# Illumina/canvas

Measured on AMD Instinct MI355X. Metric: genome-bins/sec (bin+clean+partition), higher is better.
Workload: dtype u8/int32 (bin), f32/f64 (clean, viterbi); 1 GPU; BASELINE configs[2]: whole-genome GRCh38 60x single sample, full bin+clean+partition HIP path on 1 MI355X per sample; bins_after_clean=4686240, bin_size=534, partition=PerSampleHMM, clean_flags=-g -s -r --local-sd-metric-file, segments=250, samples=1

## Files before the change

### canvas_amd/csrc/hmm.hip

```cpp
#include "common.hpp"
#include <type_traits>
#include "select.hpp"
#include "quantize.hpp"
#include <mutex>
#include <cmath>
#include <thread>
#include <cstring>
#include <limits>
#include <algorithm>

#define NSTATE 5

struct HmmParams {
    double logA[NSTATE][NSTATE];
    double logPi[NSTATE];
    int32_t tableLen;
    double maxThreshold;
};

__global__ void __launch_bounds__(256) k_keys_cov_f32(const double* __restrict__ cov, int64_t n, uint32_t* __restrict__ keys) {
    int64_t i = (int64_t)blockIdx.x * 256 + threadIdx.x;
    if (i < n) keys[i] = key_of_float((float)cov[i]);
}

// ... 232 lines not shown
            e = eNext;
        }
        __syncthreads();
        if (l < steps)
            psi[C.begin + t0 + l] = (uint16_t)(sPsi[0][l] | (sPsi[1][l] << 3) | (sPsi[2][l] << 6) | (sPsi[3][l] << 9) | (sPsi[4][l] << 12));
        __syncthreads();
    }
    double d[NSTATE];
#pragma unroll
    for (int i = 0; i < NSTATE; i++) d[i] = readlane_f64(delta, i);
    if (l == 0) {
        int best = -1; double m1 = NEG;
#pragma unroll
        for (int i = 0; i < NSTATE; i++) if (d[i] > m1) { best = i; m1 = d[i]; }
        lastState[cidx] = best;
    }
}


#define VB 128
#define VW0 16
#define VW 128
#define VW2 64
#define PQ 8
#define MAP_IDENT (0u | (1u << 3) | (2u << 6) | (3u << 9) | (4u << 12))
struct VitBlock { int32_t chrom; int32_t t0; };
struct __attribute__((aligned(4))) VecI4 { int v[4]; };
struct __attribute__((aligned(8))) VecD2 { double v[2]; };
struct __attribute__((aligned(2))) VecH8 { uint32_t w[4]; };

template <int J, bool TWO = false>
__device__ __forceinline__ void vit_state(const double (&d)[NSTATE], double e, const HmmParams& P, double& outDelta, uint32_t& outArg) {
    const double NEG = -1.7976931348623157e308;
    const double cOff = e + P.logA[J == 0 ? 1 : 0][J], cDiag = e + P.logA[J][J];
    const double t_0 = d[0] + (TWO ? (J == 0 ? cDiag : cOff) : (e + P.logA[0][J]));
    const double t_1 = d[1] + (TWO ? (J == 1 ? cDiag : cOff) : (e + P.logA[1][J]));
    const double t_2 = d[2] + (TWO ? (J == 2 ? cDiag : cOff) : (e + P.logA[2][J]));
    const double t_3 = d[3] + (TWO ? (J == 3 ? cDiag : cOff) : (e + P.logA[3][J]));
    const double t_4 = d[4] + (TWO ? (J == 4 ? cDiag : cOff) : (e + P.logA[4][J]));
    double a = __builtin_fmax(__builtin_fmax(__builtin_fmax(t_0, t_1), __builtin_fmax(t_2, t_3)), t_4);
    uint32_t ia = t_3 == a ? 3u : 4u;
    ia = t_2 == a ? 2u : ia; ia = t_1 == a ? 1u : ia; ia = t_0 == a ? 0u : ia;
    if (!(a > NEG)) { a = NEG; ia = 0; }
    outDelta = a; outArg = ia;
}
template <bool TWO = false>
__device__ __forceinline__ uint32_t vit_step5(double (&d)[NSTATE], const double (&e)[NSTATE], const HmmParams& P) {
    double n0, n1, n2, n3, n4; uint32_t a0, a1, a2, a3, a4;
    vit_state<0, TWO>(d, e[0], P, n0, a0); vit_state<1, TWO>(d, e[1], P, n1, a1); vit_state<2, TWO>(d, e[2], P, n2, a2);
    vit_state<3, TWO>(d, e[3], P, n3, a3); vit_state<4, TWO>(d, e[4], P, n4, a4);
    d[0] = n0; d[1] = n1; d[2] = n2; d[3] = n3; d[4] = n4;
    return a0 | (a1 << 3) | (a2 << 6) | (a3 << 9) | (a4 << 12);
}
__device__ __forceinline__ void vit_init5(double (&d)[NSTATE], const double (&e)[NSTATE], const HmmParams& P) {
#pragma unroll
    for (int j = 0; j < NSTATE; j++) { double lik = e[j] + P.logA[0][j]; d[j] = P.logPi[j] + lik - P.logA[0][j]; }
}
__device__ __forceinline__ int vit_best5(const double (&d)[NSTATE]) {
    int best = -1; double m1 = -1.7976931348623157e308;
#pragma unroll
    for (int i = 0; i < NSTATE; i++) if (d[i] > m1) { best = i; m1 = d[i]; }
    return best;
}
__device__ __forceinline__ uint32_t map_get(uint32_t m, uint32_t j) { return (m >> (3u * j)) & 7u; }
__device__ __forceinline__ uint32_t map_compose(uint32_t outer, uint32_t inner) {
    return map_get(outer, map_get(inner, 0)) | (map_get(outer, map_get(inner, 1)) << 3) | (map_get(outer, map_get(inner, 2)) << 6) |
           (map_get(outer, map_get(inner, 3)) << 9) | (map_get(outer, map_get(inner, 4)) << 12);
}
__device__ __forceinline__ double sel5(const double (&d)[NSTATE], uint32_t i) {
    double r = d[0];
    r = i == 1 ? d[1] : r; r = i == 2 ? d[2] : r; r = i == 3 ? d[3] : r; r = i == 4 ? d[4] : r;
    return r;
}
__device__ __forceinline__ void vit_emissions(double (&e)[NSTATE], const double* __restrict__ sTab, const double* __restrict__ logPmf, bool useLds, int tableLen, int k) {
    if (useLds) {
#pragma unroll
        for (int j = 0; j < NSTATE; j++) e[j] = sTab[k * NSTATE + j];
    } else {
#pragma unroll
        for (int j = 0; j < NSTATE; j++) e[j] = logPmf[(size_t)j * tableLen + k];
    }
}
__device__ __forceinline__ void vit_stage_table(double* sTab, const double* __restrict__ logPmf, int tableLen, bool useLds) {
    if (useLds) for (int i = threadIdx.x; i < tableLen * NSTATE; i += blockDim.x) { int s = i / tableLen, k = i - s * tableLen; sTab[k * NSTATE + s] = logPmf[i]; }
    __syncthreads();
}
__device__ __forceinline__ int wave_max_i32(int v) {
#pragma unroll
    for (int d = 32; d >= 1; d >>= 1) { int o = __shfl_xor(v, d); v = o > v ? o : v; }
    return v;
}

template <typename T>
__global__ void __launch_bounds__(256) k_make_blocks(const int32_t* __restrict__ first, int nchr, int n, int per, T* __restrict__ out) {
    const int i = blockIdx.x * 256 + threadIdx.x;
    if (i >= n) return;
    int lo = 0, hi = nchr - 1;
    while (lo < hi) { int mid = (lo + hi + 1) >> 1; if (first[mid] <= i) lo = mid; else hi = mid - 1; }
    while (lo < nchr - 1 && first[lo + 1] <= i) lo++;
    T b; b.chrom = lo; b.t0 = (i - first[lo]) * per;
    out[i] = b;
}

template <typename T> __device__ __forceinline__ void make_block_entry(const int32_t* __restrict__ first, int nchr, int i, int per, T* __restrict__ out) {
    int lo = 0, hi = nchr - 1;
    while (lo < hi) { int mid = (lo + hi + 1) >> 1; if (first[mid] <= i) lo = mid; else hi = mid - 1; }
    while (lo < nchr - 1 && first[lo + 1] <= i) lo++;
    T b; b.chrom = lo; b.t0 = (i - first[lo]) * per;
    out[i] = b;
}
#define HMM_BYVAL 64
struct HmmDescPack { HmmChrom chroms[HMM_BYVAL]; int64_t off[HMM_BYVAL + 1]; int32_t first[HMM_BYVAL + 1], firstChunk[HMM_BYVAL + 1], firstS[HMM_BYVAL + 1], firstGroup[HMM_BYVAL + 1]; };
struct HmmDescDev { HmmChrom* chroms; int64_t* off; int32_t* first; int32_t* firstChunk; int32_t* firstS; int32_t* firstGroup; };
template <typename VB_T, typename BB_T>
__global__ void __launch_bounds__(256) k_hmm_setup(const HmmDescPack pack, int usePack, HmmDescDev D, int nchr,
                                                   int nblocks, int nblocksS, int nchunks, int vb, int vbs, int bbChunk, VB_T* __restrict__ vBlocks, VB_T* __restrict__ sBlocks, BB_T* __restrict__ bChunks,
                                                   const double* __restrict__ cov, int64_t N, double maxThreshold, int32_t* __restrict__ idx, int32_t* __restrict__ dLast, int32_t* __restrict__ dFail) {
    const int32_t* first = usePack ? pack.first : D.first; const int32_t* firstS = usePack ? pack.firstS : D.firstS; const int32_t* firstChunk = usePack ? pack.firstChunk : D.firstChunk;
    if (usePack && blockIdx.x == 0) {
        for (int c = threadIdx.x; c < nchr; c += 256) D.chroms[c] = pack.chroms[c];
        for (int c = threadIdx.x; c <= nchr; c += 256) { D.off[c] = pack.off[c]; D.first[c] = pack.first[c]; D.firstChunk[c] = pack.firstChunk[c]; D.firstS[c] = pack.firstS[c]; D.firstGroup[c] = pack.firstGroup[c]; }
    }
    const int64_t i = (int64_t)blockIdx.x * 256 + threadIdx.x;
    if (i < nblocks) make_block_entry(first, nchr, (int)i, vb, vBlocks);
    if (i < nblocksS) make_block_entry(firstS, nchr, (int)i, vbs, sBlocks);
    if (i < nchunks) make_block_entry(firstChunk, nchr, (int)i, bbChunk, bChunks);
    if (i < nchr) { dLast[i] = -1; dFail[i] = 0; }
    if (cov && i < N) {
        double x = cov[i];
        x = x > maxThreshold ? maxThreshold : x;
        const int32_t k = (int32_t)rint(x);
        idx[i] = k < 0 ? 0 : k;
    }
}

template <bool useLds, bool TWO>
__global__ void __launch_bounds__(64) k_vit_spec(const VitBlock* __restrict__ blocks, int nblocks, const HmmChrom* __restrict__ chroms, const int32_t* __restrict__ idx,
                                                 const double* __restrict__ logPmf, HmmParams P, uint16_t* __restrict__ psi, uint16_t* __restrict__ maps,
                                                 int32_t* __restrict__ lastGuess, int leadIn, const int32_t* __restrict__ todo, int vb) {
    extern __shared__ double sTab[];
    vit_stage_table(sTab, logPmf, P.tableLen, useLds);
    const int b = blockIdx.x * 64 + threadIdx.x;
    const bool actBlock = b < nblocks;
    const VitBlock B = blocks[actBlock ? b : nblocks - 1];
    const HmmChrom C = chroms[B.chrom];
    const int64_t tBeg = B.t0, tEnd = (B.t0 + vb < C.T) ? B.t0 + vb : C.T;
    const int64_t ts = tBeg > leadIn ? tBeg - leadIn : 0;
    const bool act = actBlock && (!todo || todo[B.chrom]);
    const int nsteps = act ? (int)(tEnd - ts) : 0;
    const int maxSteps = wave_max_i32(nsteps);
    const int32_t* __restrict__ ix = idx + C.begin + ts;
    uint16_t* __restrict__ pp = psi + C.begin;
    double d[NSTATE] = {0.0, 0.0, 0.0, 0.0, 0.0};
    uint32_t fm = MAP_IDENT;
    const int lead = (int)(tBeg - ts);
    if (nsteps > 0) {
        double e[NSTATE];
        vit_emissions(e, sTab, logPmf, useLds, P.tableLen, ix[0]);
        if (ts == 0) vit_init5(d, e, P);
        else {
#pragma unroll
            for (int j = 0; j < NSTATE; j++) d[j] = e[j];
        }
        if (lead == 0) pp[ts] = 0;
    }
    VecI4 qa = *reinterpret_cast<const VecI4*>(ix + 1), qb = *reinterpret_cast<const VecI4*>(ix + 5);
    double eCur[NSTATE];
// ... 446 lines not shown
    double r = x0;
    r = p == 1 ? x1 : r; r = p == 2 ? x2 : r; r = p == 3 ? x3 : r; r = p == 4 ? x4 : r;
    return r;
}
struct VerState { double d[NSTATE]; uint32_t valid; bool bad; double Dprev; int sPrev; uint32_t why; };
template <bool useLds>
__device__ __forceinline__ void ver_lead_step(VerState& S, const LogA25& A, const double* __restrict__ sTab, const double* __restrict__ logPmf, int tableLen,
                                              bool on, int k, int sCur, double v, uint32_t pk) {
    double e[NSTATE];
    vit_emissions(e, sTab, logPmf, useLds, tableLen, on ? k : 0);
    const double Dt = S.Dprev + v;
    double nd[NSTATE]; uint32_t nv = 0;
    const double la5[NSTATE] = {pick5(map_get(pk, 0), LOGA_COL(A, 0)), pick5(map_get(pk, 1), LOGA_COL(A, 1)), pick5(map_get(pk, 2), LOGA_COL(A, 2)),
                                pick5(map_get(pk, 3), LOGA_COL(A, 3)), pick5(map_get(pk, 4), LOGA_COL(A, 4))};
#pragma unroll
    for (int j = 0; j < NSTATE; j++) {
        const uint32_t p = map_get(pk, j);
        const double dp = pick5(p, S.d[0], S.d[1], S.d[2], S.d[3], S.d[4]);
        const bool vp = ((S.valid >> p) & 1u) != 0;
        const double step = e[j] + la5[j];
        const bool isCur = j == sCur, fromPrev = (int)p == S.sPrev;
        const double viaPrev = S.Dprev + step, viaAnc = dp + step;
        const double r0 = vp ? viaAnc : S.d[j], r1 = fromPrev ? viaPrev : r0, r = isCur ? Dt : r1;
        nd[j] = r; nv |= (isCur || fromPrev || vp) ? (1u << j) : 0u;
    }
#pragma unroll
    for (int j = 0; j < NSTATE; j++) S.d[j] = on ? nd[j] : S.d[j];
    S.valid = on ? nv : S.valid; S.Dprev = on ? Dt : S.Dprev; S.sPrev = on ? sCur : S.sPrev;
}
template <bool useLds>
__device__ __forceinline__ void ver_block_step(VerState& S, const HmmParams& P, const double* __restrict__ sTab, const double* __restrict__ logPmf, bool on, int k, int sCur,
                                               double v, uint32_t pk) {
    double e[NSTATE], dn[NSTATE];
    vit_emissions(e, sTab, logPmf, useLds, P.tableLen, on ? k : 0);
    const double Dt = S.Dprev + v;
#pragma unroll
    for (int j = 0; j < NSTATE; j++) dn[j] = S.d[j];
    const uint32_t got = vit_step5(dn, e, P);
    S.bad = S.bad || (on && (S.valid != 31u || got != pk || sel5(dn, (uint32_t)(on ? sCur : 0)) != Dt));
    S.why |= on ? ((S.valid != 31u ? 2u : 0u) | (got != pk ? 4u : 0u) | (sel5(dn, (uint32_t)(on ? sCur : 0)) != Dt ? 8u : 0u)) : 0u;
#pragma unroll
    for (int j = 0; j < NSTATE; j++) S.d[j] = on ? dn[j] : S.d[j];
    S.Dprev = on ? Dt : S.Dprev; S.sPrev = on ? sCur : S.sPrev;
}
template <bool useLds, bool LEAD>
__device__ __forceinline__ void ver_phase(VerState& S, const LogA25& A, const HmmParams& P, const double* __restrict__ sTab, const double* __restrict__ logPmf,
                                          const int32_t* __restrict__ ixp, const int32_t* __restrict__ stp, const double* __restrict__ vp, const uint16_t* __restrict__ ppp, int cnt) {
    const int maxCnt = wave_max_i32(cnt);
    int kq[PQ], sq[PQ]; double vq[PQ]; uint32_t pq[PQ];
#pragma unroll
    for (int u = 0; u < PQ; u++) { const bool in = u < cnt; kq[u] = in ? ixp[u] : 0; sq[u] = in ? stp[u] : 0; vq[u] = in ? vp[u] : 0.0; pq[u] = in ? ppp[u] : 0u; }
    for (int j0 = 0; j0 < maxCnt; j0 += PQ) {
        int kn[PQ], sn[PQ]; double vn[PQ]; VecH8 pn;
        if (j0 + 2 * PQ <= cnt) {
            const int o = j0 + PQ;
            const VecI4 ka = *reinterpret_cast<const VecI4*>(ixp + o), kb = *reinterpret_cast<const VecI4*>(ixp + o + 4);
            const VecI4 sa = *reinterpret_cast<const VecI4*>(stp + o), sb = *reinterpret_cast<const VecI4*>(stp + o + 4);
            const VecD2 v0 = *reinterpret_cast<const VecD2*>(vp + o), v1 = *reinterpret_cast<const VecD2*>(vp + o + 2), v2 = *reinterpret_cast<const VecD2*>(vp + o + 4),
                        v3 = *reinterpret_cast<const VecD2*>(vp + o + 6);
            pn = *reinterpret_cast<const VecH8*>(ppp + o);
#pragma unroll
            for (int u = 0; u < 4; u++) { kn[u] = ka.v[u]; kn[4 + u] = kb.v[u]; sn[u] = sa.v[u]; sn[4 + u] = sb.v[u]; }
            vn[0] = v0.v[0]; vn[1] = v0.v[1]; vn[2] = v1.v[0]; vn[3] = v1.v[1]; vn[4] = v2.v[0]; vn[5] = v2.v[1]; vn[6] = v3.v[0]; vn[7] = v3.v[1];
        } else {
#pragma unroll
            for (int u = 0; u < PQ; u++) { const bool in = j0 + PQ + u < cnt; kn[u] = in ? ixp[j0 + PQ + u] : 0; sn[u] = in ? stp[j0 + PQ + u] : 0; vn[u] = in ? vp[j0 + PQ + u] : 0.0; }
#pragma unroll
            for (int u = 0; u < 4; u++) pn.w[u] = (uint32_t)(j0 + PQ + 2 * u < cnt ? ppp[j0 + PQ + 2 * u] : (uint16_t)0) | ((uint32_t)(j0 + PQ + 2 * u + 1 < cnt ? ppp[j0 + PQ + 2 * u + 1] : (uint16_t)0) << 16);
        }
#pragma unroll
        for (int u = 0; u < PQ; u++) {
            if (LEAD) ver_lead_step<useLds>(S, A, sTab, logPmf, P.tableLen, j0 + u < cnt, kq[u], sq[u], vq[u], pq[u]);
            else ver_block_step<useLds>(S, P, sTab, logPmf, j0 + u < cnt, kq[u], sq[u], vq[u], pq[u]);
        }
        __builtin_amdgcn_sched_barrier(0);
#pragma unroll
        for (int u = 0; u < PQ; u++) { kq[u] = kn[u]; sq[u] = sn[u]; vq[u] = vn[u]; pq[u] = (pn.w[u >> 1] >> (16 * (u & 1))) & 0xFFFFu; }
    }
}
template <bool useLds>
__global__ void __launch_bounds__(64) k_vit_verify(const VitBlock* __restrict__ blocks, int nblocks, const HmmChrom* __restrict__ chroms, const int32_t* __restrict__ idx,
                                                   const double* __restrict__ logPmf, HmmParams P, const uint16_t* __restrict__ psi,
                                                   const int32_t* __restrict__ state, const double* __restrict__ V, const double* __restrict__ carry, const int32_t* __restrict__ lastGuess,
                                                   int32_t* __restrict__ fail, int leadIn, const int32_t* __restrict__ todo) {
    extern __shared__ double sTab[];
    vit_stage_table(sTab, logPmf, P.tableLen, useLds);
    const int b = blockIdx.x * 64 + threadIdx.x;
    const bool actBlock = b < nblocks;
    const VitBlock B = blocks[actBlock ? b : nblocks - 1];
    const HmmChrom C = chroms[B.chrom];
    const int64_t tBeg = B.t0, tEnd = (B.t0 + VB < C.T) ? B.t0 + VB : C.T;
    const int64_t ts = tBeg > leadIn ? tBeg - leadIn : 0;
    const bool act = actBlock && (!todo || todo[B.chrom]);
    const int nsteps = act ? (int)(tEnd - ts) : 0;
    const int maxSteps = wave_max_i32(nsteps);
    const int32_t* __restrict__ ix = idx + C.begin + ts;
    const int32_t* __restrict__ st = state + C.begin + ts;
    const double* __restrict__ Vc = V + C.begin + ts;
    const uint16_t* __restrict__ pp = psi + C.begin + ts;
    VerState S;
#pragma unroll
    for (int j = 0; j < NSTATE; j++) S.d[j] = 0.0;
    S.valid = 0; S.bad = false; S.why = 0;
    S.Dprev = carry[C.begin + ts];
    S.sPrev = ts > 0 ? state[C.begin + ts - 1] : -1;
    LogA25 A;
#define LOGA_LOAD(i, j) A.a##i##j = P.logA[i][j]; asm volatile("" : "+v"(A.a##i##j));
    LOGA_LOAD(0, 0) LOGA_LOAD(0, 1) LOGA_LOAD(0, 2) LOGA_LOAD(0, 3) LOGA_LOAD(0, 4) LOGA_LOAD(1, 0) LOGA_LOAD(1, 1) LOGA_LOAD(1, 2) LOGA_LOAD(1, 3) LOGA_LOAD(1, 4)
    LOGA_LOAD(2, 0) LOGA_LOAD(2, 1) LOGA_LOAD(2, 2) LOGA_LOAD(2, 3) LOGA_LOAD(2, 4) LOGA_LOAD(3, 0) LOGA_LOAD(3, 1) LOGA_LOAD(3, 2) LOGA_LOAD(3, 3) LOGA_LOAD(3, 4)
    LOGA_LOAD(4, 0) LOGA_LOAD(4, 1) LOGA_LOAD(4, 2) LOGA_LOAD(4, 3) LOGA_LOAD(4, 4)
#undef LOGA_LOAD
    const int lead = (int)(tBeg - ts);
    if (nsteps > 0) {
        if (ts == 0) {
            double e[NSTATE];
            vit_emissions(e, sTab, logPmf, useLds, P.tableLen, ix[0]);
            const double Dt = S.Dprev + Vc[0];
            const int sCur = st[0];
            vit_init5(S.d, e, P); S.valid = 31u;
            if (sel5(S.d, (uint32_t)sCur) != Dt) { S.bad = true; S.why |= 16u; }
            S.Dprev = Dt; S.sPrev = sCur;
        } else ver_lead_step<useLds>(S, A, sTab, logPmf, P.tableLen, true, ix[0], st[0], Vc[0], (uint32_t)pp[0]);
    }
    const int start2 = lead > 1 ? lead : 1;
    ver_phase<useLds, true>(S, A, P, sTab, logPmf, ix + 1, st + 1, Vc + 1, pp + 1, nsteps > 0 && lead > 1 ? lead - 1 : 0);
    ver_phase<useLds, false>(S, A, P, sTab, logPmf, ix + start2, st + start2, Vc + start2, pp + start2, nsteps > start2 ? nsteps - start2 : 0);
    double (&d)[NSTATE] = S.d; const uint32_t valid = S.valid; bool bad = S.bad;
    uint32_t why = S.why;
    if (act && tEnd == C.T) { if (valid != 31u || vit_best5(d) != lastGuess[B.chrom]) { bad = true; why |= 32u; } }
    if (act && bad) atomicOr(&fail[B.chrom], (int32_t)(1u | why));
}

__global__ void k_vit_corrupt(uint16_t* __restrict__ psi, int64_t at) {
    if (threadIdx.x == 0 && blockIdx.x == 0) { uint32_t v = psi[at], p = (v >> 6) & 7u; psi[at] = (uint16_t)((v & ~(7u << 6)) | (((p + 1u) % 5u) << 6)); }
}

__global__ void __launch_bounds__(256) k_bt_maps(const VitBlock* __restrict__ blocks, int nblocks, const HmmChrom* __restrict__ chroms, const uint16_t* __restrict__ psi,
                                                 uint16_t* __restrict__ maps) {
    int b = blockIdx.x * 256 + threadIdx.x;
    if (b >= nblocks) return;
    const VitBlock B = blocks[b];
    const HmmChrom C = chroms[B.chrom];
    const int64_t tBeg = B.t0 > 0 ? B.t0 : 1, tEnd = (B.t0 + VB < C.T) ? B.t0 + VB : C.T;
    uint32_t m = MAP_IDENT;
    for (int64_t t = tEnd - 1; t >= tBeg; t--) m = map_compose(psi[C.begin + t], m);
    maps[b] = (uint16_t)m;
}
__global__ void __launch_bounds__(64) k_bt_group(const int32_t* __restrict__ firstBlock, const int32_t* __restrict__ firstGroup, int nchr, const uint16_t* __restrict__ maps,
                                                 uint16_t* __restrict__ pre, uint16_t* __restrict__ gmap) {
    const int g = blockIdx.x, l = threadIdx.x;
    int lo = 0, hi = nchr - 1;
    while (lo < hi) { const int mid = (lo + hi + 1) >> 1; if (firstGroup[mid] <= g) lo = mid; else hi = mid - 1; }
    while (lo < nchr - 1 && firstGroup[lo + 1] <= g) lo++;
    const int first = firstBlock[lo], last = firstBlock[lo + 1] - 1;
    const int bi = last - ((g - firstGroup[lo]) * 64 + l);
    uint32_t f = bi >= first ? (uint32_t)maps[bi] : MAP_IDENT;
#pragma unroll
    for (int dlt = 1; dlt < 64; dlt <<= 1) { const uint32_t o = __shfl_up(f, dlt); if (l >= dlt) f = map_compose(f, o); }
    const uint32_t ex = __shfl_up(f, 1);
    if (bi >= first) pre[bi] = (uint16_t)(l == 0 ? MAP_IDENT : ex);
    if (l == 63) gmap[g] = (uint16_t)f;
}
__global__ void __launch_bounds__(64) k_bt_gchain(const int32_t* __restrict__ firstGroup, const int32_t* __restrict__ lastState, const uint16_t* __restrict__ gmap,
                                                  int8_t* __restrict__ gentry) {
    const int c = blockIdx.x, l = threadIdx.x;
    const int g0 = firstGroup[c], ng = firstGroup[c + 1] - g0;
    int s = lastState[c];
    for (int base = 0; base < ng; base += 64) {
        uint32_t f = base + l < ng ? (uint32_t)gmap[g0 + base + l] : MAP_IDENT;
#pragma unroll
        for (int dlt = 1; dlt < 64; dlt <<= 1) { const uint32_t o = __shfl_up(f, dlt); if (l >= dlt) f = map_compose(f, o); }
        const uint32_t ex = __shfl_up(f, 1);
        if (base + l < ng) gentry[g0 + base + l] = (int8_t)(s < 0 ? s : (l == 0 ? s : (int)map_get(ex, (uint32_t)s)));
        const uint32_t all = (uint32_t)__builtin_amdgcn_readlane((int)f, 63);
        if (s >= 0) s = (int)map_get(all, (uint32_t)s);
    }
// ... 306 lines not shown
    std::vector<int32_t> firstGroup(nchr + 1);
    int ngroups = 0;
    for (int c = 0; c < nchr; c++) { firstGroup[c] = ngroups; ngroups += (firstBlock[c + 1] - firstBlock[c] + 63) / 64; }
    firstGroup[nchr] = ngroups;
    std::vector<int32_t> firstS(nchr + 1);
    int nblocksS = 0;
    for (int c = 0; c < nchr; c++) { firstS[c] = nblocksS; if (chroms[c].T > 10) nblocksS += (int)((chroms[c].T + VBS - 1) / VBS); }
    firstS[nchr] = nblocksS;
    std::vector<int32_t> firstChunk(nchr + 1);
    int nchunks = 0;
    for (int c = 0; c < nchr; c++) {
        firstChunk[c] = nchunks;
        if (chroms[c].T > 10) nchunks += (int)((chroms[c].T + BB_CHUNK - 1) / BB_CHUNK);
    }
    firstChunk[nchr] = nchunks;
    const int nbSeg = (int)nblk2(N, 2048);
    WsSizer sz;
    sz.take<BbChunk>(nchunks + 1); sz.take<int32_t>(nchr + 1); sz.take<double>(nchunks + 1); sz.take<double>(nchunks + 1); sz.take<BbChunkOut>(nchunks + 1);
    sz.take<BbCross>((size_t)nchunks * BB_MAXC + 1); sz.take<ParFn>((size_t)nchunks * 16 + 1); sz.take<uint8_t>((size_t)nchunks * 16 + 8);
    sz.take<unsigned long long>(nchunks + 1); sz.take<BbPost>((size_t)nchunks * BB_MAXC + 1);
    sz.take<uint16_t>(N + 8); sz.take<HmmChrom>(nchr); sz.take<int32_t>(nchr);
    sz.take<int32_t>(nchr + 1); sz.take<uint16_t>(nblocks + 8); sz.take<int8_t>(nblocks + 8);
    sz.take<int64_t>(nchr + 1); sz.take<VitBlock>(nblocks + 1); sz.take<double>(N); sz.take<double>(N + 64); sz.take<int32_t>(nchr); sz.take<int32_t>(nchr);
    sz.take<VitBlock>(nblocksS + 1); sz.take<uint16_t>(nblocksS + 8); sz.take<int32_t>(nchr + 1);
    sz.take<int32_t>(nchr + 1); sz.take<uint16_t>(nblocks + 8); sz.take<uint16_t>(ngroups + 8); sz.take<int8_t>(ngroups + 8);
    sz.take<char>(8 * 256 + (size_t)nchr * 64 + 64);
    if (seg) { sz.take<uint8_t>(N + 16); sz.take<uint32_t>(nbSeg + 1); sz.take<unsigned long long>(1); }
    int32_t rc = canvas_ws_reserve(ctx, sz.off + extraBytes + 65536); if (rc) return rc;
    rc = canvas_pin_reserve(ctx, (size_t)nchr * 4 + 64); if (rc) return rc;
    WsCarver ws(ctx->ws);
    uint16_t* psi = ws.take<uint16_t>(N + 8);
    HmmChrom* dChroms = ws.take<HmmChrom>(nchr); int32_t* dLast = ws.take<int32_t>(nchr);
    int32_t* dFirst = ws.take<int32_t>(nchr + 1);
    uint16_t* dMaps = ws.take<uint16_t>(nblocks + 8); (void)ws.take<int8_t>(nblocks + 8);
    int64_t* dOffDev = ws.take<int64_t>(nchr + 1);
    VitBlock* dVBlocks = ws.take<VitBlock>(nblocks + 1); double* dD = ws.take<double>(N); double* dCarry = ws.take<double>(N + 64); int32_t* dFail = ws.take<int32_t>(nchr); int32_t* dRedo = ws.take<int32_t>(nchr);
    int32_t* dFirstGroup = ws.take<int32_t>(nchr + 1); uint16_t* dPre = ws.take<uint16_t>(nblocks + 8); uint16_t* dGmap = ws.take<uint16_t>(ngroups + 8);
    int8_t* dGentry = ws.take<int8_t>(ngroups + 8);
    VitBlock* dSBlocks = ws.take<VitBlock>(nblocksS + 1); uint16_t* dMapsS = ws.take<uint16_t>(nblocksS + 8); int32_t* dFirstS = ws.take<int32_t>(nchr + 1);
    BbChunk* dBChunks = ws.take<BbChunk>(nchunks + 1); int32_t* dFirstChunk = ws.take<int32_t>(nchr + 1);
    double* dChunkSum = ws.take<double>(nchunks + 1); double* dChunkBase = ws.take<double>(nchunks + 1); BbChunkOut* dChunkOut = ws.take<BbChunkOut>(nchunks + 1);
    BbCross* dCross = ws.take<BbCross>((size_t)nchunks * BB_MAXC + 1); ParFn* dAt64Fn = ws.take<ParFn>((size_t)nchunks * 16 + 1); uint8_t* dAt64Rank = ws.take<uint8_t>((size_t)nchunks * 16 + 8);
    unsigned long long* dChunkBits = ws.take<unsigned long long>(nchunks + 1); BbPost* dPost = ws.take<BbPost>((size_t)nchunks * BB_MAXC + 1);
    uint8_t* segFlags = nullptr; uint32_t* segBlockCnt = nullptr; unsigned long long* segTot = nullptr;
    if (seg) { segFlags = ws.take<uint8_t>(N + 16); segBlockCnt = ws.take<uint32_t>(nbSeg + 1); segTot = ws.take<unsigned long long>(1); seg->valid = false; }

    const bool byVal = descByValue && nchr <= HMM_BYVAL;
    HmmDescPack pack;
    {
        auto al = [](size_t v) { return (v + 255) & ~size_t(255); };
        const size_t oCh = 0, oFirst = al((size_t)nchr * sizeof(HmmChrom)), oOff = oFirst + al((size_t)(nchr + 1) * 4), oChunk = oOff + al((size_t)(nchr + 1) * 8),
                     oS = oChunk + al((size_t)(nchr + 1) * 4), oG = oS + al((size_t)(nchr + 1) * 4), total = oG + al((size_t)(nchr + 1) * 4);
        char* dBlob = ws.take<char>(total);
        if (byVal) {
            memset(&pack, 0, sizeof pack);
            memcpy(pack.chroms, chroms.data(), (size_t)nchr * sizeof(HmmChrom)); memcpy(pack.off, h_chr_offset, (size_t)(nchr + 1) * 8); memcpy(pack.first, firstBlock.data(), (size_t)(nchr + 1) * 4);
            memcpy(pack.firstChunk, firstChunk.data(), (size_t)(nchr + 1) * 4); memcpy(pack.firstS, firstS.data(), (size_t)(nchr + 1) * 4); memcpy(pack.firstGroup, firstGroup.data(), (size_t)(nchr + 1) * 4);
        } else {
            std::vector<char> blob(total, 0);
            memcpy(blob.data() + oCh, chroms.data(), (size_t)nchr * sizeof(HmmChrom)); memcpy(blob.data() + oFirst, firstBlock.data(), (size_t)(nchr + 1) * 4);
            memcpy(blob.data() + oOff, h_chr_offset, (size_t)(nchr + 1) * 8); memcpy(blob.data() + oChunk, firstChunk.data(), (size_t)(nchr + 1) * 4);
            memcpy(blob.data() + oS, firstS.data(), (size_t)(nchr + 1) * 4); memcpy(blob.data() + oG, firstGroup.data(), (size_t)(nchr + 1) * 4);
            rc = canvas_h2d_small(ctx, dBlob, blob.data(), total); if (rc) return rc;
        }
        dChroms = (HmmChrom*)(dBlob + oCh); dFirst = (int32_t*)(dBlob + oFirst); dOffDev = (int64_t*)(dBlob + oOff); dFirstChunk = (int32_t*)(dBlob + oChunk);
        dFirstS = (int32_t*)(dBlob + oS); dFirstGroup = (int32_t*)(dBlob + oG);
    }
    HmmParams P; HmmEmis E;
    ctx->hmm_dispersion = 1e9;
    rc = prepareA(ws, P, E, (const HmmChrom*)dChroms, (const int64_t*)dOffDev); if (rc) return rc;
    {
        const int64_t most = std::max<int64_t>(std::max<int64_t>(E.indexCov ? N : 0, nblocks), std::max<int64_t>(std::max(nblocksS, nchunks), nchr));
        HmmDescDev DD{dChroms, dOffDev, dFirst, dFirstChunk, dFirstS, dFirstGroup};
        hipLaunchKernelGGL((k_hmm_setup<VitBlock, BbChunk>), dim3(nblk2(most, 256)), dim3(256), 0, ctx->stream, pack, byVal ? 1 : 0, DD, nchr, nblocks, nblocksS, nchunks, VB, VBS, BB_CHUNK,
                           dVBlocks, dSBlocks, dBChunks, E.indexCov, N, P.maxThreshold, E.idx, dLast, dFail);
    }
    rc = prepareB(ws, P, E); if (rc) return rc;
    int32_t* idx = E.idx; double* dTab = E.dTab;
    size_t tabBytes = (size_t)NSTATE * P.tableLen * 8;
    size_t lds = tabBytes <= 48 * 1024 ? tabBytes : 0;
    for (int c = 0; c < nchr; c++)
        if (chroms[c].T <= 10 && chroms[c].T > 0)
            hipLaunchKernelGGL(k_fill_i32, dim3(nblk2(chroms[c].T, 256)), dim3(256), 0, ctx->stream, d_state, chroms[c].begin, chroms[c].begin + chroms[c].T, -1);
    const unsigned laneGrid = (unsigned)((nblocks + 63) / 64);
    auto backtrack = [&](bool haveMaps) {
        if (nblocks > 0) {
            if (!haveMaps) hipLaunchKernelGGL(k_bt_maps, dim3(nblk2(nblocks, 256)), dim3(256), 0, ctx->stream, dVBlocks, nblocks, dChroms, psi, dMaps);
            hipLaunchKernelGGL(k_bt_group, dim3(ngroups), dim3(64), 0, ctx->stream, dFirst, dFirstGroup, nchr, dMaps, dPre, dGmap);
            hipLaunchKernelGGL(k_bt_gchain, dim3(nchr), dim3(64), 0, ctx->stream, dFirstGroup, dLast, dGmap, dGentry);
            hipLaunchKernelGGL(k_bt_states, dim3(nblk2(nblocks, 4)), dim3(256), 0, ctx->stream, dVBlocks, nblocks, dChroms, psi, dFirst, dFirstGroup, dPre, dGentry, d_state);
        }
    };
    bool twoValuedAll = true;
    for (int i = 0; i < NSTATE; i++) for (int j = 0; j < NSTATE; j++) {
        const double ref = i == j ? P.logA[0][0] : P.logA[0][1];
        if (memcmp(&P.logA[i][j], &ref, sizeof(double)) != 0) twoValuedAll = false;
    }
    const bool speculative = cvx_hook("CANVAS_HMM_SEQUENTIAL") == nullptr;
    std::vector<int32_t> redo;
    int32_t* hFail = (int32_t*)ctx->pin; unsigned long long* hSegTot = (unsigned long long*)((char*)ctx->pin + (((size_t)nchr * 4 + 15) & ~size_t(15)));
    bool segEnqueued = false; unsigned* hSegSeq = (unsigned*)(hSegTot + 1); unsigned segSeq = 0;
    if (speculative && nblocks > 0) {
        ProfScope ps(ctx, "viterbi");
        const int32_t* dTodo = nullptr;
        ctx->hmm_retry = 0;
        static const int vwEnv = cvx_hook("CANVAS_HMM_LEAD") ? atoi(cvx_hook("CANVAS_HMM_LEAD")) : 0;
        const int vw0 = vwEnv > 0 ? vwEnv : (ctx->hmm_dispersion < 0.20 ? VW0 : (ctx->hmm_dispersion < 0.30 ? 64 : VW));
        const int nAttempts = 5;
        for (int attempt = 0; attempt < nAttempts; attempt++) {
            const int mult = attempt <= 1 ? 1 : (attempt == 2 ? 8 : (attempt == 3 ? 64 : 512));
            const int leadSpec = attempt == 0 ? vw0 : mult * VW, leadVer = mult * VW2;
            if (attempt > 0) CANVAS_HIP_TRY(ctx, hipMemsetAsync(dFail, 0, nchr * 4, ctx->stream));
            const dim3 gs((unsigned)((nblocksS + 63) / 64));
            const bool twoValued = twoValuedAll && attempt < 3;
            if (lds && twoValued) hipLaunchKernelGGL((k_vit_spec<true, true>), gs, dim3(64), lds, ctx->stream, dSBlocks, nblocksS, dChroms, idx, dTab, P, psi, dMapsS, dLast, leadSpec, dTodo, VBS);
            else if (lds) hipLaunchKernelGGL((k_vit_spec<true, false>), gs, dim3(64), lds, ctx->stream, dSBlocks, nblocksS, dChroms, idx, dTab, P, psi, dMapsS, dLast, leadSpec, dTodo, VBS);
            else if (twoValued) hipLaunchKernelGGL((k_vit_spec<false, true>), gs, dim3(64), 0, ctx->stream, dSBlocks, nblocksS, dChroms, idx, dTab, P, psi, dMapsS, dLast, leadSpec, dTodo, VBS);
            else hipLaunchKernelGGL((k_vit_spec<false, false>), gs, dim3(64), 0, ctx->stream, dSBlocks, nblocksS, dChroms, idx, dTab, P, psi, dMapsS, dLast, leadSpec, dTodo, VBS);
            hipLaunchKernelGGL(k_pair_maps, dim3(nblk2(nblocks, 256)), dim3(256), 0, ctx->stream, dVBlocks, nblocks, dChroms, dFirstS, dMapsS, dMaps, dTodo);
            if (attempt == 0 && cvx_hook("CANVAS_HMM_TEST_CORRUPT")) hipLaunchKernelGGL(k_vit_corrupt, dim3(1), dim3(64), 0, ctx->stream, psi, chroms[0].begin + chroms[0].T / 2);
            backtrack(true);
            hipLaunchKernelGGL(k_vit_increments, dim3(nblk2(N, 256)), dim3(256), 0, ctx->stream, dChroms, nchr, dOffDev, idx, dTab, P, d_state, N, dD);
            const char* bbMode = cvx_hook("CANVAS_HMM_BACKBONE");
            if ((bbMode && !strcmp(bbMode, "chain")) || (attempt > 1 && !bbMode)) hipLaunchKernelGGL(k_vit_backbone, dim3(nchr), dim3(64), 0, ctx->stream, dChroms, dD, dCarry, dTodo);
            else if (bbMode && !strcmp(bbMode, "scan")) hipLaunchKernelGGL(k_vit_backbone_scan, dim3(nchr), dim3(BS_T), 0, ctx->stream, dChroms, dD, dCarry, dFail);
            else {
                hipLaunchKernelGGL(k_bb_sums, dim3(nchunks), dim3(256), 0, ctx->stream, dBChunks, dChroms, dD, dChunkSum, dFail);
                hipLaunchKernelGGL(k_bb_bases, dim3(nchr), dim3(64), 0, ctx->stream, dFirstChunk, dChunkSum, dChunkBase);
                hipLaunchKernelGGL(k_bb_pieces, dim3(nchunks), dim3(256), 0, ctx->stream, dBChunks, dChroms, dD, dChunkBase, dChunkOut, dCross, dAt64Fn, dAt64Rank, dFail);
                hipLaunchKernelGGL(k_bb_walk, dim3(nchr), dim3(64), 0, ctx->stream, dFirstChunk, dChunkOut, dCross, dChunkBits, dPost, dFail);
                hipLaunchKernelGGL(k_bb_emit, dim3(nblk2((int64_t)nchunks * 16, 256)), dim3(256), 0, ctx->stream, dBChunks, nchunks, dChroms, dChunkBits, dPost, dAt64Fn, dAt64Rank, dCarry);
            }
            if (lds) hipLaunchKernelGGL((k_vit_verify<true>), dim3(laneGrid), dim3(64), lds, ctx->stream, dVBlocks, nblocks, dChroms, idx, dTab, P, psi, d_state, dD, dCarry, dLast, dFail, leadVer, dTodo);
            else hipLaunchKernelGGL((k_vit_verify<false>), dim3(laneGrid), dim3(64), 0, ctx->stream, dVBlocks, nblocks, dChroms, idx, dTab, P, psi, d_state, dD, dCarry, dLast, dFail, leadVer, dTodo);
            CANVAS_HIP_TRY(ctx, hipMemcpyAsync(hFail, dFail, nchr * 4, hipMemcpyDeviceToHost, ctx->stream));
            if (seg && attempt == 0 && !cvx_hook("CANVAS_HMM_TEST_CORRUPT")) {
                (void)segTot;
                segSeq = cvx_mail_arm(ctx, hSegSeq);
                enqueue_segment_ids(ctx, dOffDev, nchr, d_state, seg->d_start, seg->d_stop, N, seg->maxDist, segFlags, segBlockCnt, hSegTot , seg->d_segment_id, hSegSeq, segSeq);
                segEnqueued = true;
            }
            CANVAS_HIP_TRY(ctx, hipStreamSynchronize(ctx->stream));
            redo.clear();
            for (int c = 0; c < nchr; c++) if (hFail[c] && chroms[c].T > 10) redo.push_back(c);
            if (!redo.empty() && cvx_hook("CANVAS_HMM_DEBUG_FAIL")) { fprintf(stderr, "viterbi attempt %d (lead-in x%d):", attempt, mult); for (int c : redo) fprintf(stderr, " chr%d(T=%lld, why=0x%x)", c, (long long)chroms[c].T, (unsigned)hFail[c]); fprintf(stderr, "\n"); }
            if (redo.empty() || cvx_hook("CANVAS_HMM_TEST_CORRUPT") || cvx_hook("CANVAS_HMM_NO_RETRY")) break;
            if (attempt < nAttempts - 1) {
                if (attempt == 0) { ctx->hmm_retry = (int)redo.size(); { ProfScope pr(ctx, "viterbi_retry"); } }
                int32_t rcq = canvas_h2d_small(ctx, dRedo, hFail, nchr * 4); if (rcq) return rcq;
                dTodo = dRedo;
            }
        }
        if (seg && segEnqueued && redo.empty() && ctx->hmm_retry == 0) { int32_t rcm = cvx_mail_await(ctx, hSegSeq, segSeq, "PerSampleHMM: segment count"); if (rcm) return rcm; seg->valid = true; seg->nseg = (int64_t)*hSegTot; }
    } else {
        for (int c = 0; c < nchr; c++) redo.push_back(c);
    }
    if (!redo.empty()) {
        const bool isFallback = speculative && nblocks > 0;
        ProfScope ps(ctx, isFallback ? "viterbi_sequential" : "viterbi_small");
        if (cvx_hook("CANVAS_HMM_DEBUG_FAIL")) { fprintf(stderr, "viterbi sequential kernel for %zu chromosomes (speculative %d, blocks %d):", redo.size(), (int)speculative, nblocks); for (size_t i = 0; i < redo.size() && i < 6; i++) fprintf(stderr, " chr%d(T=%lld)", redo[i], (long long)chroms[redo[i]].T); fprintf(stderr, "\n"); }
        rc = canvas_h2d_small(ctx, dRedo, redo.data(), redo.size() * 4); if (rc) return rc;
        hipLaunchKernelGGL(k_viterbi, dim3((unsigned)redo.size()), dim3(64), lds, ctx->stream, dChroms, idx, dTab, P, psi, dLast, dRedo);
        backtrack(false);
    }
    ctx->hmm_redo = (int)redo.size();
    CANVAS_HIP_TRY(ctx, hipStreamSynchronize(ctx->stream));
    CANVAS_HIP_TRY(ctx, hipGetLastError());
    return CANVAS_OK;
}

extern "C" {

static int32_t hmm_per_sample_impl(canvas_ctx* ctx, int32_t nchr, const double* d_cov, const int64_t* h_chr_offset, const double* d_cov_all, int64_t nAll, int32_t* d_state, const CovQ* preQ = nullptr, SegPost* seg = nullptr) {
    if (!ctx) return CANVAS_ERR_INVALID;
    if (nchr <= 0 || !d_cov || !h_chr_offset || !d_state || !d_cov_all) CANVAS_FAIL(ctx, CANVAS_ERR_INVALID, "canvas_hmm_per_sample: bad arguments");
    CANVAS_HIP_TRY(ctx, hipSetDevice(ctx->device));
    const int64_t N = h_chr_offset[nchr];
    if (nAll < 5) CANVAS_FAIL(ctx, CANVAS_ERR_UNSUPPORTED, "HMM: fewer than 5 bins genome-wide (Quartiles would throw in the reference)");
    WsSizer ex; ex.take<uint32_t>(nAll); ex.take<int32_t>(N + 256); ex.take<double>(NSTATE * 70000); ex.take<CovQ>(1); ex.take<uint32_t>(CQ_WIN);
    double haploidMean = 0, pseudoVariance = 0;
    std::vector<double> tab;
    struct Joiner { NbPool* p = nullptr; ~Joiner() { if (p) p->finish(); } } joiner;
    auto prepareA = [&](WsCarver& ws, HmmParams& P, HmmEmis& E, const HmmChrom*, const int64_t*) -> int32_t {
        int32_t rc;
        uint32_t* keys = ws.take<uint32_t>(nAll); int32_t* idx = ws.take<int32_t>(N + 256); double* dTab = ws.take<double>(NSTATE * 70000);
    int64_t qidx[6]; int nq;
    quartile_idx(nAll, qidx, nq);
    float v[6], q1, q2, q3;
    bool radix = cvx_hook("CANVAS_HMM_RADIX_SELECT") != nullptr;
    if (!radix && preQ) { rc = cvx_mail_await(ctx, &preQ->pad, ctx->covq_seq, "PerSampleHMM: coverage quartiles"); if (rc) return rc; }
    if (!radix && preQ && preQ->nq == (uint32_t)nq && preQ->n == nAll) {
        bool same = true; for (int k = 0; k < nq; k++) same = same && preQ->rank[k] == (unsigned long long)qidx[k];
        if (same && !preQ->bad && !preQ->fail) for (int k = 0; k < nq; k++) v[k] = (float)((double)preQ->resultK[k] / 100.0);
        else radix = true;
    } else if (!radix) {
        CovQ* dQ = ws.take<CovQ>(1); uint32_t* dWin = ws.take<uint32_t>(CQ_WIN);
        CovQ hQ; memset(&hQ, 0, sizeof hQ); hQ.nq = (uint32_t)nq;
        for (int k = 0; k < nq; k++) hQ.rank[k] = (unsigned long long)qidx[k];
        rc = canvas_h2d_small(ctx, dQ, &hQ, sizeof hQ); if (rc) return rc;
        CANVAS_HIP_TRY(ctx, hipMemsetAsync(dWin, 0, CQ_WIN * 4, ctx->stream));
        hipLaunchKernelGGL(k_covq_hist, dim3(256), dim3(1024), 0, ctx->stream, d_cov_all, nAll, dQ, dWin);
        hipLaunchKernelGGL(k_covq_pick, dim3(1), dim3(1024), 0, ctx->stream, dQ, dWin);
        rc = canvas_pin_reserve(ctx, sizeof(CovQ)); if (rc) return rc;
        CANVAS_HIP_TRY(ctx, hipMemcpyAsync(ctx->pin, dQ, sizeof(CovQ), hipMemcpyDeviceToHost, ctx->stream));
        CANVAS_HIP_TRY(ctx, hipStreamSynchronize(ctx->stream));
        CANVAS_HIP_TRY(ctx, hipGetLastError());
        const CovQ& R = *(const CovQ*)ctx->pin;
        if (R.bad || R.fail) radix = true;
        else for (int k = 0; k < nq; k++) v[k] = (float)((double)R.resultK[k] / 100.0);
    }
    if (radix) {
        hipLaunchKernelGGL(k_keys_cov_f32, dim3(nblk2(nAll, 256)), dim3(256), 0, ctx->stream, d_cov_all, nAll, keys);
        std::vector<SelQuery> qs;
        for (int k = 0; k < nq; k++) qs.push_back({0, 0, qidx[k]});
        std::vector<unsigned long long> res;
        rc = radix_select<uint32_t>(ctx, keys, 1, std::vector<int64_t>{0, nAll}, qs, res); if (rc) return rc;
        for (int k = 0; k < nq; k++) v[k] = host_float_of_key((uint32_t)res[k]);
// ... 299 lines not shown
```

Measured before the change: 2.012 billion bins/s.

## Split Viterbi verify blocks across sub-lanes and restage emission table coalesced

The verify kernel can now split each Viterbi block across several lanes (two on the first attempt when dispersion is low). Each lane checks a shorter sub-range with its own lead-in, which shortens the serial per-lane walk and increases the number of lanes in flight. The LDS staging of the emission table is also restructured so each thread loads whole rows of five states over four unrolled positions, replacing a per-element divide. The trade-off is more total lead-in work and a dependence on the dispersion estimate, which before this point is set to 1e9, so the split may never trigger.

```diff
diff --git a/canvas_amd/csrc/hmm.hip b/canvas_amd/csrc/hmm.hip
--- a/canvas_amd/csrc/hmm.hip
+++ b/canvas_amd/csrc/hmm.hip
@@ -338,7 +338,18 @@
     }
 }
 __device__ __forceinline__ void vit_stage_table(double* sTab, const double* __restrict__ logPmf, int tableLen, bool useLds) {
-    if (useLds) for (int i = threadIdx.x; i < tableLen * NSTATE; i += blockDim.x) { int s = i / tableLen, k = i - s * tableLen; sTab[k * NSTATE + s] = logPmf[i]; }
+    if (useLds) for (int k0 = threadIdx.x; k0 < tableLen; k0 += 4 * blockDim.x) {
+        double v[4][NSTATE];
+#pragma unroll
+        for (int u = 0; u < 4; u++) { const int k = k0 + u * (int)blockDim.x;
+#pragma unroll
+            for (int s = 0; s < NSTATE; s++) v[u][s] = k < tableLen ? logPmf[(size_t)s * tableLen + k] : 0.0; }
+#pragma unroll
+        for (int u = 0; u < 4; u++) { const int k = k0 + u * (int)blockDim.x;
+            if (k < tableLen) {
+#pragma unroll
+                for (int s = 0; s < NSTATE; s++) sTab[k * NSTATE + s] = v[u][s]; } }
+    }
     __syncthreads();
 }
 __device__ __forceinline__ int wave_max_i32(int v) {
@@ -951,16 +962,18 @@
 __global__ void __launch_bounds__(64) k_vit_verify(const VitBlock* __restrict__ blocks, int nblocks, const HmmChrom* __restrict__ chroms, const int32_t* __restrict__ idx,
                                                    const double* __restrict__ logPmf, HmmParams P, const uint16_t* __restrict__ psi,
                                                    const int32_t* __restrict__ state, const double* __restrict__ V, const double* __restrict__ carry, const int32_t* __restrict__ lastGuess,
-                                                   int32_t* __restrict__ fail, int leadIn, const int32_t* __restrict__ todo) {
+                                                   int32_t* __restrict__ fail, int leadIn, const int32_t* __restrict__ todo, int sub) {
     extern __shared__ double sTab[];
     vit_stage_table(sTab, logPmf, P.tableLen, useLds);
-    const int b = blockIdx.x * 64 + threadIdx.x;
+    const int r = blockIdx.x * 64 + threadIdx.x;
+    const int b = r / sub, h = r - b * sub, vr = VB / sub;
     const bool actBlock = b < nblocks;
     const VitBlock B = blocks[actBlock ? b : nblocks - 1];
     const HmmChrom C = chroms[B.chrom];
-    const int64_t tBeg = B.t0, tEnd = (B.t0 + VB < C.T) ? B.t0 + VB : C.T;
+    const bool inChrom = (int64_t)B.t0 + (int64_t)h * vr < C.T;
+    const int64_t tBeg = inChrom ? (int64_t)B.t0 + (int64_t)h * vr : (int64_t)B.t0, tEnd = (tBeg + vr < C.T) ? tBeg + vr : C.T;
     const int64_t ts = tBeg > leadIn ? tBeg - leadIn : 0;
-    const bool act = actBlock && (!todo || todo[B.chrom]);
+    const bool act = actBlock && inChrom && (!todo || todo[B.chrom]);
     const int nsteps = act ? (int)(tEnd - ts) : 0;
     const int maxSteps = wave_max_i32(nsteps);
     const int32_t* __restrict__ ix = idx + C.begin + ts;
@@ -1433,7 +1446,6 @@
     for (int c = 0; c < nchr; c++)
         if (chroms[c].T <= 10 && chroms[c].T > 0)
             hipLaunchKernelGGL(k_fill_i32, dim3(nblk2(chroms[c].T, 256)), dim3(256), 0, ctx->stream, d_state, chroms[c].begin, chroms[c].begin + chroms[c].T, -1);
-    const unsigned laneGrid = (unsigned)((nblocks + 63) / 64);
     auto backtrack = [&](bool haveMaps) {
         if (nblocks > 0) {
             if (!haveMaps) hipLaunchKernelGGL(k_bt_maps, dim3(nblk2(nblocks, 256)), dim3(256), 0, ctx->stream, dVBlocks, nblocks, dChroms, psi, dMaps);
@@ -1482,8 +1494,10 @@
                 hipLaunchKernelGGL(k_bb_walk, dim3(nchr), dim3(64), 0, ctx->stream, dFirstChunk, dChunkOut, dCross, dChunkBits, dPost, dFail);
                 hipLaunchKernelGGL(k_bb_emit, dim3(nblk2((int64_t)nchunks * 16, 256)), dim3(256), 0, ctx->stream, dBChunks, nchunks, dChroms, dChunkBits, dPost, dAt64Fn, dAt64Rank, dCarry);
             }
-            if (lds) hipLaunchKernelGGL((k_vit_verify<true>), dim3(laneGrid), dim3(64), lds, ctx->stream, dVBlocks, nblocks, dChroms, idx, dTab, P, psi, d_state, dD, dCarry, dLast, dFail, leadVer, dTodo);
-            else hipLaunchKernelGGL((k_vit_verify<false>), dim3(laneGrid), dim3(64), 0, ctx->stream, dVBlocks, nblocks, dChroms, idx, dTab, P, psi, d_state, dD, dCarry, dLast, dFail, leadVer, dTodo);
+            const int verSub = (attempt == 0 && ctx->hmm_dispersion < 0.30) ? 2 : 1;
+            const unsigned verGrid = (unsigned)(((int64_t)nblocks * verSub + 63) / 64);
+            if (lds) hipLaunchKernelGGL((k_vit_verify<true>), dim3(verGrid), dim3(64), lds, ctx->stream, dVBlocks, nblocks, dChroms, idx, dTab, P, psi, d_state, dD, dCarry, dLast, dFail, leadVer, dTodo, verSub);
+            else hipLaunchKernelGGL((k_vit_verify<false>), dim3(verGrid), dim3(64), 0, ctx->stream, dVBlocks, nblocks, dChroms, idx, dTab, P, psi, d_state, dD, dCarry, dLast, dFail, leadVer, dTodo, verSub);
             CANVAS_HIP_TRY(ctx, hipMemcpyAsync(hFail, dFail, nchr * 4, hipMemcpyDeviceToHost, ctx->stream));
             if (seg && attempt == 0 && !cvx_hook("CANVAS_HMM_TEST_CORRUPT")) {
                 (void)segTot;
```

Result: faster. 2.033 billion bins/s, median of 6 (+1.1%).
